# FHE-ACCELE/Homulator

Hardware: AMD Instinct MI355X
Metric: hmult+key-switch ops/sec (higher is better)
Workload: dtype u64

## Files before the change

homulator_amd/csrc/hm_backend.hip:

```cpp
#include <hip/hip_runtime.h>
#include <dlfcn.h>
#include <rccl/rccl.h>
#include <algorithm>
#include <cstdarg>
#include <cstdio>
#include <cstring>
#include <map>
#include <tuple>
#include <type_traits>
#include <utility>
#include <memory>
#include <stdexcept>
#include <string>
#include <vector>

#include "../../include/homulator_hip.h"
#include "hm_elem_core.h"
#include "hm_ip_core.h"
#include "hm_modarith.h"
#include "hm_ntt_core.h"
#include "hm_params.h"
#include "hm_caps.h"
#include "hm_launch.h"
#include "hm_bconv_plan.h"


__device__ __forceinline__ bool hm_block_map(uint32_t tiles_per_limb, uint32_t n_entries, uint32_t logG, uint32_t &entry, uint32_t &tile) {
  const uint32_t b = blockIdx.x, xcd = b & 7u, slot = b >> 3;
  const uint32_t per = tiles_per_limb << logG;
  const uint32_t grp = slot / per, within = slot % per;
  tile = within >> logG;
  entry = grp * (8u << logG) + (within & ((1u << logG) - 1u)) * 8u + xcd;
  return entry < n_entries;
}

#ifndef HM_ROW_WAVE_SYNC
#define HM_ROW_WAVE_SYNC 0
#endif
template <bool STRIDED>
__device__ __forceinline__ void hm_pass_sync(int nth) {
  if (STRIDED || !HM_ROW_WAVE_SYNC || nth == 0) __syncthreads();
  else { __builtin_amdgcn_fence(__ATOMIC_ACQ_REL, "wavefront"); __builtin_amdgcn_wave_barrier(); }
}

struct Geo16 {
  static constexpr int EPT = 16;
  typedef hm16::HmNttState State;
  template <int TL, int LOGR, bool STRIDED> static constexpr int ldsWords() { return hm16::HmLds<TL, LOGR, STRIDED>::WORDS; }
  template <int TL, int LOGR, bool STRIDED, bool INV, int MODE, int LDAUX, int STAUX, int EPICH, class... A>
  static __device__ __forceinline__ void phases(A &&...a) { hm16::hm_ntt_pass_phases<TL, LOGR, STRIDED, INV, MODE, LDAUX, STAUX, EPICH>(a...); }
};
struct Geo8 {
  static constexpr int EPT = 8;
  typedef hm8::HmNttState State;
  template <int TL, int LOGR, bool STRIDED> static constexpr int ldsWords() { return hm8::HmLds<TL, LOGR, STRIDED>::WORDS; }
  template <int TL, int LOGR, bool STRIDED, bool INV, int MODE, int LDAUX, int STAUX, int EPICH, class... A>
  static __device__ __forceinline__ void phases(A &&...a) { hm8::hm_ntt_pass_phases<TL, LOGR, STRIDED, INV, MODE, LDAUX, STAUX, EPICH>(a...); }
};
template <int LOGR, bool STRIDED, bool INV, int MODE, int LDAUX = 0, int STAUX = 0, int EPICH = HM_EPI_CHUNK, class GEO = Geo16, class PRE = HmNoPre>
__device__ __forceinline__ void hm_ntt_pass_run(const HmNttArgs &a, uint64_t *lds, uint32_t entry, uint32_t tile, int tid, PRE pre = PRE()) {
  constexpr int TL = HM_TL(STRIDED);
  const HmLimb lb = a.limb[entry];
  const uint32_t mod = lb.mod;
  const size_t N = (size_t)1 << a.logN;
  const uint64_t q = HM_CONST_MODS(a.mods)[mod].q;
  const HmW *twl = a.tw + (size_t)mod * N;
  const uint32_t s0 = STRIDED ? 0u : (a.logN - HM_ROW_LOG);
  const uint32_t prefix0 = STRIDED ? 0u : (tile << (TL - LOGR));
  const HmW *twt = STRIDED ? nullptr : a.twist + ((size_t)mod * (N >> HM_ROW_LOG) + prefix0) * 3;
  constexpr bool FIRST = (STRIDED != INV);
  const uint64_t *src = FIRST ? a.in + (size_t)lb.in * N : a.out + (size_t)lb.out * N;
  uint64_t *dst = a.out + (size_t)lb.out * N;

  HmTw sc = {0, 0};
  HmEpi ep = hm_epi_none();
  typedef const HmNttEntry __attribute__((address_space(4))) *ConstEntry;
  const ConstEntry entries = (ConstEntry)(uintptr_t)a.entry;
  if constexpr (MODE == 2) { sc.w = entries[entry].sc.w; sc.ws = entries[entry].sc.ws; ep.pack = entries[entry].pack; }
  if constexpr (MODE == 3 || MODE == 7) {
    const auto &en = entries[entry];
    sc.w = en.sc.w; sc.ws = en.sc.ws;
    ep.a = a.minuend + (size_t)lb.aux * N;
    ep.d = a.addend && en.alimb != HM_NTT_NONE ? a.addend + (size_t)en.alimb * N : nullptr;
    ep.dk.w = en.ak.w; ep.dk.ws = en.ak.ws;
    if constexpr (MODE == 7) { ep.g = en.galois; ep.logN = a.logN; }
  }
  if constexpr (MODE == 6) { ep.g = entries[entry].galois; ep.logN = a.logN; }
  if constexpr (MODE == 4) {
    const auto &en = entries[entry];
    ep.b = a.mix + (size_t)en.mixlimb * N;
    ep.bk.w = en.mixk.w; ep.bk.ws = en.mixk.ws;
  }
  typename GEO::State st;
  int nsync = 0;
  GEO::template phases<TL, LOGR, STRIDED, INV, MODE, LDAUX, STAUX, EPICH>(st, tid, lds, src, dst, tile, twl, twt, s0, prefix0, q, sc, ep,
                                                                           [&] { hm_pass_sync<STRIDED>(nsync++); }, pre);
}

template <int LOGR, bool STRIDED, bool INV, int MODE, class GEO = Geo16>
__device__ __forceinline__ void hm_ntt_pass_body(const HmNttArgs &a) {
  constexpr int TL = HM_TL(STRIDED);
  __shared__ __attribute__((aligned(16))) uint64_t lds[GEO::template ldsWords<TL, LOGR, STRIDED>()];
  uint32_t entry, tile;
  if (!hm_block_map(1u << (a.logN - TL), a.n_limbs, a.logG, entry, tile)) return;
  if (a.limb[entry].mod == HM_NTT_NONE) return;
#if defined(HM_ABL_EMPTY)
  return;
#endif
  hm_ntt_pass_run<LOGR, STRIDED, INV, MODE, 0, 0, HM_EPI_CHUNK, GEO>(a, lds, entry, tile, threadIdx.x);
}

#ifndef HM_NTT_MIN_WAVES
#define HM_NTT_MIN_WAVES 4
#endif
#ifndef HM_NTT_MIN_WAVES_COL
#define HM_NTT_MIN_WAVES_COL HM_NTT_MIN_WAVES
#endif
template <int LOGR, bool INV, int MODE>
__global__ void __launch_bounds__((1 << HM_TL_COL) / HM_EPT) __attribute__((amdgpu_waves_per_eu(HM_NTT_MIN_WAVES_COL))) k_ntt_col(HmNttArgs a) {
  hm_ntt_pass_body<LOGR, true, INV, MODE>(a);
}
template <bool INV, int MODE>
__global__ void __launch_bounds__((1 << HM_TL_ROW) / HM_EPT) __attribute__((amdgpu_waves_per_eu(HM_NTT_MIN_WAVES))) k_ntt_row(HmNttArgs a) {
  hm_ntt_pass_body<HM_ROW_LOG, false, INV, MODE>(a);
}

template <int LOG1, bool INV, int MODE>
__global__ void __launch_bounds__((1 << HM_TL_COL) / 8) k_ntt_col8(HmNttArgs a) {
  hm_ntt_pass_body<LOG1, true, INV, MODE, Geo8>(a);
}
template <bool INV, int MODE>
__global__ void __launch_bounds__((1 << HM_TL_ROW) / 8) k_ntt_row8(HmNttArgs a) {
  hm_ntt_pass_body<HM_ROW_LOG, false, INV, MODE, Geo8>(a);
}

struct HmLimbSync {
  unsigned long long w;
  unsigned long long pad[15];
};
struct HmNttSync {
  HmLimbSync fast[HM_NTT_MAX_ENTRIES];
  unsigned long long arrive2[HM_NTT_MAX_ENTRIES];
  unsigned done[HM_NTT_MAX_ENTRIES];
  unsigned xccmask[HM_NTT_MAX_ENTRIES];
  unsigned stats[4];
};
#define HM_SPIN_LIMIT (1u << 22)
#ifndef HM_OPAQUE_TID2
#define HM_OPAQUE_TID2 1
#endif
#ifndef HM_FUSED_IN_AUX
#define HM_FUSED_IN_AUX 0
#endif
#ifndef HM_FUSED_OUT_AUX
#define HM_FUSED_OUT_AUX 0
#endif
#ifndef HM_FUSED_MID_AUX
#define HM_FUSED_MID_AUX 16
#endif
__device__ __forceinline__ unsigned hm_xcc_id() {
  unsigned v;
  asm volatile("s_getreg_b32 %0, hwreg(HW_REG_XCC_ID, 0, 4)" : "=s"(v));
  return v & 7u;
}
__device__ __forceinline__ unsigned long long hm_l2_add(unsigned long long *p, unsigned long long v) {
  unsigned long long old;
  asm volatile("global_atomic_add_x2 %0, %1, %2, off sc0\n\ts_waitcnt vmcnt(0)" : "=v"(old) : "v"(p), "v"(v) : "memory");
  return old;
}
__device__ __forceinline__ void hm_l2_zero(unsigned long long *p) {
  unsigned long long old, z = 0;
  asm volatile("global_atomic_swap_x2 %0, %1, %2, off sc0\n\ts_waitcnt vmcnt(0)" : "=v"(old) : "v"(p), "v"(z) : "memory");
}
__device__ __forceinline__ void hm_l2_add_noret(unsigned long long *p, unsigned long long v) {
  asm volatile("global_atomic_add_x2 %0, %1, off" ::"v"(p), "v"(v) : "memory");
}
__device__ __forceinline__ void hm_limb_arrive(HmNttSync *ws, uint32_t entry, bool withhold) {
  asm volatile("s_waitcnt vmcnt(0)" ::: "memory");
  __syncthreads();
  if (threadIdx.x == 0 && !withhold) hm_l2_add_noret(&ws->fast[entry].w, 1ull);
}
__device__ __forceinline__ uint32_t hm_limb_wait(HmNttSync *ws, unsigned *err, uint32_t entry, uint32_t members, uint32_t *lds_flag, uint32_t spin_limit,
    uint32_t pretend_spread = 0, uint32_t tile = 0) {
  if (threadIdx.x == 0) {
    unsigned long long *w = &ws->fast[entry].w;
    uint32_t fast = 0;
    unsigned spins = 0;
// ... 769 lines not shown
  if (g->owner) {
    if (g->owner->live_graphs > 0) g->owner->live_graphs--;
    auto &v = g->owner->graphs;
    v.erase(std::remove(v.begin(), v.end(), g), v.end());
  }
  (void)hipGraphExecDestroy(g->exec);
  (void)hipGraphDestroy(g->graph);
  delete g;
}

extern "C" hm_status hm_timer_start(hm_ctx *c) {
  if (!c) return HM_ERR_ARG;
  HM_HIP(c, hipEventRecord(c->ev0, c->stream));
  return HM_OK;
}
extern "C" hm_status hm_timer_stop(hm_ctx *c, uint64_t *ns) {
  if (!c || !ns) return HM_ERR_ARG;
  HM_HIP(c, hipEventRecord(c->ev1, c->stream));
  HM_HIP(c, hipEventSynchronize(c->ev1));
  if (hm_status st = check_device_error(c)) return st;
  float ms = 0;
  HM_HIP(c, hipEventElapsedTime(&ms, c->ev0, c->ev1));
  *ns = (uint64_t)((double)ms * 1e6);
  return HM_OK;
}

static hm_status check_limbs(hm_ctx *c, const char *what, const uint32_t *l, uint32_t n) {
  for (uint32_t i = 0; l && i < n; ++i)
    if (l[i] > 0xFFFFu) return fail(c, HM_ERR_ARG, "%s: limb index %u exceeds 65535", what, l[i]);
  return HM_OK;
}
static hm_status check_mods(hm_ctx *c, const char *what, const uint32_t *m, uint32_t n) {
  if (!m) return fail(c, HM_ERR_ARG, "%s: mod_ids is null", what);
  for (uint32_t i = 0; i < n; ++i)
    if (m[i] >= c->P.L + c->P.K) return fail(c, HM_ERR_ARG, "%s: mod id %u out of range", what, m[i]);
  return HM_OK;
}

typedef void (*hm_ntt_kernel)(HmNttArgs);
typedef void (*hm_ntt_one_kernel)(HmNttArgs, HmNttFusedArgs);
struct HmNttKernels {
  hm_ntt_kernel first, second, first8, second8;
  hm_ntt_one_kernel one[2];
};
#define HM_NTT_FORMS 6
template <int LOG1>
static const HmNttKernels &ntt_kernels(int form) {
  static const HmNttKernels wide[HM_NTT_FORMS] = {
      {k_ntt_col<LOG1, false, 0>, k_ntt_row<false, 1>, nullptr, nullptr, {nullptr, nullptr}},
      {k_ntt_col<LOG1, false, 0>, k_ntt_row<false, 3>, nullptr, nullptr, {nullptr, nullptr}},
      {k_ntt_col<LOG1, false, 4>, k_ntt_row<false, 3>, nullptr, nullptr, {nullptr, nullptr}},
      {k_ntt_row<true, 0>, k_ntt_col<LOG1, true, 2>, nullptr, nullptr, {nullptr, nullptr}},
      {k_ntt_row<true, 6>, k_ntt_col<LOG1, true, 2>, nullptr, nullptr, {nullptr, nullptr}},
      {k_ntt_col<LOG1, false, 0>, k_ntt_row<false, 7>, nullptr, nullptr, {nullptr, nullptr}}};
  return wide[form];
}
template <int LOG1>
static const HmNttKernels &ntt_kernels_all(int form) {
  static const HmNttKernels both[HM_NTT_FORMS] = {
      {k_ntt_col<LOG1, false, 0>, k_ntt_row<false, 1>, k_ntt_col8<LOG1, false, 0>, k_ntt_row8<false, 1>, {k_ntt_fused8<LOG1, false, 0, 1, true>,
          k_ntt_fused8<LOG1, false, 0, 1, false>}},
      {k_ntt_col<LOG1, false, 0>, k_ntt_row<false, 3>, k_ntt_col8<LOG1, false, 0>, k_ntt_row8<false, 3>, {k_ntt_fused8<LOG1, false, 0, 3, true>,
          k_ntt_fused8<LOG1, false, 0, 3, false>}},
      {k_ntt_col<LOG1, false, 4>, k_ntt_row<false, 3>, k_ntt_col8<LOG1, false, 4>, k_ntt_row8<false, 3>, {k_ntt_fused8<LOG1, false, 4, 3, true>,
          k_ntt_fused8<LOG1, false, 4, 3, false>}},
      {k_ntt_row<true, 0>, k_ntt_col<LOG1, true, 2>, k_ntt_row8<true, 0>, k_ntt_col8<LOG1, true, 2>, {k_ntt_fused8<LOG1, true, 0, 2, true>,
          k_ntt_fused8<LOG1, true, 0, 2, false>}},
      {k_ntt_row<true, 6>, k_ntt_col<LOG1, true, 2>, k_ntt_row8<true, 6>, k_ntt_col8<LOG1, true, 2>, {k_ntt_fused8<LOG1, true, 6, 2, true>,
          k_ntt_fused8<LOG1, true, 6, 2, true>}},
      {k_ntt_col<LOG1, false, 0>, k_ntt_row<false, 7>, k_ntt_col8<LOG1, false, 0>, k_ntt_row8<false, 7>, {k_ntt_fused8<LOG1, false, 0, 7, true>,
          k_ntt_fused8<LOG1, false, 0, 7, false>}}};
  return both[form];
}
template <> const HmNttKernels &ntt_kernels<8>(int form) { return ntt_kernels_all<8>(form); }
template <> const HmNttKernels &ntt_kernels<7>(int form) { return ntt_kernels_all<7>(form); }

static uint32_t small_entries(const hm_ctx *c, uint32_t limbs16) {
  if (!hm_caps(c->P.logN).small_geometry) return 0;
  return std::min<uint32_t>(HM_NTT_MAX_ENTRIES, limbs16 << (16 - std::min(16u, c->P.logN)));
}
static uint32_t fused_small_entries(const hm_ctx *c) { return small_entries(c, c->fused_small); }

template <int LOG1>
static void launch_ntt(hm_ctx *c, const HmNttArgs &a, int form, bool firstPassOnly, bool secondPassOnly = false) {
  const HmNttKernels &K = ntt_kernels<LOG1>(form);
  const bool inverse = form == 3 || form == 4;
  const dim3 grid(a.n_limbs * (c->P.N >> HM_TL_ROW)), block16((1 << HM_TL_ROW) / HM_EPT), block8((1 << HM_TL_ROW) / 8);
  const bool small = K.first8 && c->small_ept8 && a.n_limbs <= small_entries(c, c->small_limbs);
  const bool col8 = small && (c->small_mode & 1), row8 = small && (c->small_mode & 2);
  const bool first8 = inverse ? row8 : col8, second8 = inverse ? col8 : row8;
  if (secondPassOnly) {
    hipLaunchKernelGGL(second8 ? K.second8 : K.second, grid, second8 ? block8 : block16, 0, c->stream, a);
    return;
  }
  if (firstPassOnly) {
    hipLaunchKernelGGL(K.first, grid, block16, 0, c->stream, a);
    return;
  }
  if (K.one[0] && a.n_limbs <= fused_small_entries(c) && a.logG == 0) {
    HmNttFusedArgs f = {c->ntt_ws, c->err_dev, c->fused_test_spread, c->fused_test_timeout ? 1u << 10 : HM_SPIN_LIMIT, c->fused_test_timeout};
#if defined(HM_FUSED_TRACE)
    f.trace = c->fused_trace;
#endif
    if (c->capturing) c->capture_has_fused = true;
    bool inPlace = a.in == a.out;
    for (uint32_t e = 0; inPlace && e < a.n_limbs; ++e) inPlace = a.limb[e].mod == HM_NTT_NONE || a.limb[e].in == a.limb[e].out;
    hipLaunchKernelGGL(K.one[inPlace ? 1 : 0], grid, block8, 0, c->stream, a, f);
    return;
  }
  hipLaunchKernelGGL(first8 ? K.first8 : K.first, grid, first8 ? block8 : block16, 0, c->stream, a);
  hipLaunchKernelGGL(second8 ? K.second8 : K.second, grid, second8 ? block8 : block16, 0, c->stream, a);
}

static hm_status device_table(hm_ctx *c, const void *data, size_t bytes, const void **out) {
  const std::string key(static_cast<const char *>(data), bytes);
  auto it = c->launch_tables.find(key);
  if (it == c->launch_tables.end()) {
    hipStreamCaptureStatus cs = hipStreamCaptureStatusNone;
    if (hipStreamIsCapturing(c->stream, &cs) == hipSuccess && cs != hipStreamCaptureStatusNone)
      return fail(c, HM_ERR_UNSUPPORTED, "a launch table is missing while the stream is capturing: run the plan once before hm_capture_begin");
    if (c->launch_tables.size() >= 1024 && c->live_graphs == 0 && !c->capturing) {
      HM_HIP(c, hipStreamSynchronize(c->stream));
      for (auto &kv : c->launch_tables) (void)hipFree(kv.second);
      c->launch_tables.clear();
    }
    void *dev = nullptr;
    HM_HIP(c, hipMalloc(&dev, bytes));
    HM_HIP(c, hipMemcpy(dev, data, bytes, hipMemcpyHostToDevice));
    it = c->launch_tables.emplace(key, dev).first;
  }
  *out = it->second;
  return HM_OK;
}
static hm_status ntt_table(hm_ctx *c, const std::vector<HmNttEntry> &tab, const HmNttEntry **out) {
  const void *p = nullptr;
  hm_status st = device_table(c, tab.data(), sizeof(HmNttEntry) * tab.size(), &p);
  *out = static_cast<const HmNttEntry *>(p);
  return st;
}

struct NttFused {
  const uint64_t *minuend = nullptr;
  const uint32_t *minuend_limbs = nullptr;
  const uint64_t *addend = nullptr;
  const uint32_t *addend_limbs = nullptr;
  const uint64_t *addend_k = nullptr;
  const uint64_t *mix = nullptr;
  const uint32_t *mix_limbs = nullptr;
  const uint64_t *mix_k = nullptr;
  const uint8_t *outPacked = nullptr;
  const uint32_t *inGalois = nullptr;
  const uint32_t *addGalois = nullptr;
  bool firstPassOnly = false;
  bool secondPassOnly = false;
};

static hm_status ntt_common(hm_ctx *c, const char *what, const uint64_t *in, const uint32_t *in_limbs, uint64_t *out,
                            const uint32_t *out_limbs, const uint32_t *mod_ids, uint32_t n, int inverse, const uint64_t *k,
                            const NttFused &f) {
  const bool fused = f.minuend != nullptr;
  hm_status st;
  if ((st = check_limbs(c, what, in_limbs, n)) || (st = check_limbs(c, what, out_limbs, n)) ||
      (st = check_limbs(c, what, f.minuend_limbs, n)) ||
      (st = check_limbs(c, what, f.mix_limbs, n)) || (st = check_mods(c, what, mod_ids, n)))
    return st;
  for (uint32_t g = 0; f.addend_limbs && g < n; ++g)
    if (f.addend_limbs[g] != HM_NO_LIMB && f.addend_limbs[g] >= 0xFFFFu) return fail(c, HM_ERR_ARG, "%s: addend limb index %u exceeds 65534", what,
        f.addend_limbs[g]);
  for (uint32_t g = 0; g < n; ++g) {
    const uint64_t q = c->P.mod[mod_ids[g]];
    if ((k && k[g] >= q) || (f.addend_k && f.addend_k[g] >= q) || (f.mix_k && f.mix_k[g] >= q))
      return fail(c, HM_ERR_ARG, "%s: constant [%u] is not reduced", what, g);
    if (f.addend_k && f.addend_k[g] == 0) return fail(c, HM_ERR_ARG, "%s: addend_k[%u] is zero (pass addend = NULL instead)", what, g);
  }
  bool anyInGalois = false, anyAddGalois = false;
  for (uint32_t g = 0; g < n; ++g) {
    const uint32_t gi = f.inGalois ? f.inGalois[g] : 0, ga = f.addGalois ? f.addGalois[g] : 0;
    if ((gi && (!(gi & 1) || gi >= 2 * c->P.N)) || (ga && (!(ga & 1) || ga >= 2 * c->P.N)))
      return fail(c, HM_ERR_ARG, "%s: Galois element [%u] is not an odd number below 2N", what, g);
    anyInGalois |= gi > 1; anyAddGalois |= ga > 1;
  }
  if (anyInGalois) {
    const int64_t g = hm_first_overlap(out, out_limbs, n, in, in_limbs, n, c->P.N, [&](uint32_t i) { return f.inGalois[i] > 1; });
    if (g >= 0) return fail(c, HM_ERR_ARG,
        "%s: limb-poly [%u] is read through an automorphism from a limb the call also writes (not in place, and not onto another entry's source)", what, (uint32_t)g);
  }
  if (anyInGalois && (!inverse || f.secondPassOnly)) return fail(c, HM_ERR_ARG, "%s: only the inverse transform reads its input through an automorphism", what);
  if (anyAddGalois && (!fused || f.mix || !f.addend)) return fail(c, HM_ERR_UNSUPPORTED,
      "%s: the addend is read through an automorphism by the fused forward transform without the mix prologue only", what);
  if (anyAddGalois) {
    const int64_t g = hm_first_overlap(out, out_limbs, n, f.addend, f.addend_limbs, n, c->P.N,
        [&](uint32_t i) { return f.addGalois[i] > 1 && !(f.addend_limbs && f.addend_limbs[i] == HM_NO_LIMB); });
    if (g >= 0) return fail(c, HM_ERR_ARG, "%s: the addend of limb-poly [%u] is read through an automorphism from a limb the call writes", what, (uint32_t)g);
  }
  HM_HIP(c, hipSetDevice(c->device));
  const bool oneLaunch = fused_small_entries(c) && !f.firstPassOnly && !f.secondPassOnly && (n + 7) / 8 * 8 <= fused_small_entries(c);
  std::vector<uint32_t> all(n);
  for (uint32_t i = 0; i < n; ++i) all[i] = i;
  const HmGrouping grouping = hm_group_by_modulus(mod_ids, all, hm_ntt_group_policy(oneLaunch));
  const auto &groups = grouping.groups;
  const uint32_t logG = grouping.logG, G = 1u << logG;
  const HmLaunchSplit parts = hm_launch_split((uint32_t)groups.size(), std::min<uint32_t>(HM_NTT_MAX_ENTRIES, c->ntt_launch_entries), G);
  for (uint32_t base = 0; base < groups.size(); base += parts.perLaunch) {
    const uint32_t ng = hm_launch_groups(parts, (uint32_t)groups.size(), base), cnt = hm_launch_entries(ng, G);
    std::vector<HmNttEntry> tab(cnt);
    memset(tab.data(), 0, sizeof(HmNttEntry) * cnt);
    HmNttArgs a;
    for (uint32_t e = 0; e < cnt; ++e) a.limb[e] = HmLimb{0, 0, (uint16_t)HM_NTT_NONE, 0};
    for (uint32_t kk = 0; kk < ng; ++kk) {
      for (uint32_t which = 0; which < G; ++which) {
        const int gi = groups[base + kk][which];
        if (gi < 0) continue;
        const uint32_t g = (uint32_t)gi, e = hm_entry_slot(kk, which, G), m = mod_ids[g];
        const uint64_t q = c->P.mod[m];
        HmNttEntry &t = tab[e];
        a.limb[e] = HmLimb{(uint16_t)limb_at(in_limbs, g), (uint16_t)limb_at(out_limbs, g), (uint16_t)m, 0};
        if (inverse) {
          uint64_t v = c->P.modc[m].ninv;
          if (k) v = hm::mulmod(v, k[g], q);
          t.sc = hm_kconst(v, q);
          t.pack = f.outPacked && f.outPacked[g] ? 1 : 0;
          if (anyInGalois) t.galois = f.inGalois[g] ? f.inGalois[g] : 1u;
        } else if (fused) {
          if (anyAddGalois) t.galois = f.addGalois[g] ? f.addGalois[g] : 1u;
          t.sc = hm_kconst(k[g], q);
          a.limb[e].aux = (uint16_t)limb_at(f.minuend_limbs, g);
          t.alimb = f.addend_limbs && f.addend_limbs[g] == HM_NO_LIMB ? (uint16_t)HM_NTT_NONE : (uint16_t)limb_at(f.addend_limbs, g);
          if (f.addend_k) t.ak = hm_kconst(f.addend_k[g], q);
          if (f.mix) {
            t.mixlimb = (uint16_t)limb_at(f.mix_limbs, g);
            t.mixk = hm_kconst(f.mix_k[g], q);
          }
        }
      }
    }
    const HmNttEntry *dtab = nullptr;
    if (inverse || fused) {
      if ((st = ntt_table(c, tab, &dtab))) return st;
    }
    a.in = in; a.out = out;
    a.tw = inverse ? c->d_tw_inv : c->d_tw_fwd;
    a.twist = inverse ? c->d_twist_inv : c->d_twist_fwd;
    a.mods = c->d_mods;
    a.entry = dtab;
    a.minuend = f.minuend; a.addend = f.addend; a.mix = f.mix;
    a.logN = c->P.logN; a.n_limbs = cnt; a.logG = logG;
    const int form = inverse ? (anyInGalois ? 4 : 3) : fused ? (f.mix ? 2 : anyAddGalois ? 5 : 1) : 0;
    static void (*const launch[])(hm_ctx *, const HmNttArgs &, int, bool, bool) = {launch_ntt<5>, launch_ntt<6>, launch_ntt<7>, launch_ntt<8>, launch_ntt<9>};
    const uint32_t log1 = c->P.logN - HM_ROW_LOG;
    if (log1 < 5 || log1 > 9) return fail(c, HM_ERR_UNSUPPORTED, "%s: logN %u", what, c->P.logN);
    launch[log1 - 5](c, a, form, f.firstPassOnly, f.secondPassOnly);
    HM_HIP(c, hipGetLastError());
  }
  return HM_OK;
}

extern "C" hm_status hm_ntt(hm_ctx *c, const uint64_t *in, const uint32_t *in_limbs, uint64_t *out,
                            const uint32_t *out_limbs, const uint32_t *mod_ids, uint32_t n, int inverse,
                            const uint64_t *scale) {
  if (!c) return HM_ERR_ARG;
  if (!in || !out) return fail(c, HM_ERR_ARG, "hm_ntt: null buffer");
  if (scale && !inverse) return fail(c, HM_ERR_ARG, "hm_ntt: scale is only defined for the inverse transform");
  return ntt_common(c, "hm_ntt", in, in_limbs, out, out_limbs, mod_ids, n, inverse, scale, NttFused{});
}

extern "C" hm_status hm_ntt_second_pass(hm_ctx *c, uint64_t *buf, const uint32_t *limbs, const uint32_t *mod_ids, uint32_t n, int inverse,
                                        const uint64_t *scale) {
  if (!c) return HM_ERR_ARG;
  if (!buf) return fail(c, HM_ERR_ARG, "hm_ntt_second_pass: null buffer");
  if (scale && !inverse) return fail(c, HM_ERR_ARG, "hm_ntt_second_pass: scale is only defined for the inverse transform");
  NttFused f;
  f.secondPassOnly = true;
  return ntt_common(c, "hm_ntt_second_pass", buf, limbs, buf, limbs, mod_ids, n, inverse, scale, f);
}

extern "C" hm_status hm_ntt_ex(hm_ctx *c, const hm_ntt_desc *d) {
  if (!c) return HM_ERR_ARG;
  if (!d || !d->out || (!d->in && !d->second_pass_only)) return fail(c, HM_ERR_ARG, "hm_ntt_ex: null buffer");
  if (d->scale && !d->inverse) return fail(c, HM_ERR_ARG, "hm_ntt_ex: scale is only defined for the inverse transform");
  if (d->out_packed && !d->inverse) return fail(c, HM_ERR_ARG, "hm_ntt_ex: out_packed is only defined for the inverse transform");
  NttFused f;
  f.secondPassOnly = d->second_pass_only != 0;
  f.outPacked = d->out_packed;
  f.inGalois = d->in_galois;
  if (d->in_galois && !d->inverse) return fail(c, HM_ERR_ARG, "hm_ntt_ex: in_galois is only defined for the inverse transform");
  if (f.secondPassOnly) return ntt_common(c, "hm_ntt_ex", d->out, d->out_limbs, d->out, d->out_limbs, d->mod_ids, d->n, d->inverse, d->scale, f);
  return ntt_common(c, "hm_ntt_ex", d->in, d->in_limbs, d->out, d->out_limbs, d->mod_ids, d->n, d->inverse, d->scale, f);
}

extern "C" hm_status hm_ntt_sub_scale(hm_ctx *c, const uint64_t *in, const uint32_t *in_limbs, const uint64_t *minuend,
                                      const uint32_t *minuend_limbs, const uint64_t *addend, const uint32_t *addend_limbs,
                                      uint64_t *out, const uint32_t *out_limbs, const uint32_t *mod_ids, uint32_t n,
                                      const uint64_t *k) {
  if (!c) return HM_ERR_ARG;
  if (!in || !out || !minuend || !k) return fail(c, HM_ERR_ARG, "hm_ntt_sub_scale: null argument");
  NttFused f;
  f.minuend = minuend; f.minuend_limbs = minuend_limbs; f.addend = addend; f.addend_limbs = addend_limbs;
  return ntt_common(c, "hm_ntt_sub_scale", in, in_limbs, out, out_limbs, mod_ids, n, 0, k, f);
}

struct BcolMix {
  const uint64_t *mix;
  const uint32_t *const *mix_limbs;
  const uint64_t *const *mix_k;
};
static hm_status bconv_col_launch(hm_ctx *c, const hm_bconv_desc *descs, uint32_t n_desc, const BcolMix *mix, uint32_t tile0 = 0, uint32_t n_tiles = 0);
extern "C" hm_status hm_ntt_mix_sub_scale(hm_ctx *c, const hm_ntt_fused_desc *d) {
  if (!c) return HM_ERR_ARG;
  if (!d || (!d->in && !d->n_conv) || !d->out || !d->minuend || !d->k) return fail(c, HM_ERR_ARG, "hm_ntt_mix_sub_scale: null argument");
  if ((d->mix != nullptr) != (d->mix_k != nullptr)) return fail(c, HM_ERR_ARG, "hm_ntt_mix_sub_scale: mix and mix_k go together");
  if (d->addend_k && !d->addend) return fail(c, HM_ERR_ARG, "hm_ntt_mix_sub_scale: addend_k without addend");
  NttFused f;
  f.minuend = d->minuend; f.minuend_limbs = d->minuend_limbs; f.addend = d->addend; f.addend_limbs = d->addend_limbs;
  f.addend_k = d->addend_k; f.mix = d->mix; f.mix_limbs = d->mix_limbs; f.mix_k = d->mix_k;
  f.addGalois = d->addend_galois;
  if (d->addend_galois && (d->n_conv || d->mix || !d->addend)) return fail(c, HM_ERR_UNSUPPORTED,
      "hm_ntt_mix_sub_scale: addend_galois needs an addend and combines with neither the mix prologue nor conversions inside the transform");
  if (!d->n_conv) return ntt_common(c, "hm_ntt_mix_sub_scale", d->in, d->in_limbs, d->out, d->out_limbs, d->mod_ids, d->n, 0, d->k, f);
  if (!d->conv) return fail(c, HM_ERR_ARG, "hm_ntt_mix_sub_scale: n_conv without descriptors");
  const uint32_t n = d->n;
  std::map<uint32_t, uint32_t> byOut;
  for (uint32_t i = 0; i < n; ++i)
    if (!byOut.emplace(limb_at(d->out_limbs, i), i).second) return fail(c, HM_ERR_ARG, "hm_ntt_mix_sub_scale: output limb %u appears twice",
        limb_at(d->out_limbs, i));
  std::vector<char> covered(n, 0);
  std::vector<std::vector<uint32_t>> mixLimbs(d->n_conv);
  std::vector<std::vector<uint64_t>> mixK(d->n_conv);
  std::vector<const uint32_t *> mlp(d->n_conv);
  std::vector<const uint64_t *> mkp(d->n_conv);
  for (uint32_t j = 0; j < d->n_conv; ++j) {
    const hm_bconv_desc &cv = d->conv[j];
    if (cv.out != d->out) return fail(c, HM_ERR_ARG, "hm_ntt_mix_sub_scale: conv[%u].out must be the output buffer", j);
    if (!cv.out_ids || cv.n_out == 0 || cv.n_out > HM_BCONV_MAX_OUT) return fail(c, HM_ERR_ARG, "hm_ntt_mix_sub_scale: conv[%u]: bad output basis", j);
    for (uint32_t t = 0; t < cv.n_out; ++t) {
// ... 422 lines not shown
```

homulator_amd/csrc/hm_launch.h:

```cpp
#pragma once
#include <algorithm>
#include <cstdint>
#include <map>
#include <vector>

static inline uint32_t limb_at(const uint32_t *l, uint32_t i) { return l ? l[i] : i; }

static inline uint32_t hm_entry_slot(uint32_t kk, uint32_t which, uint32_t G) { return (kk / 8) * 8 * G + which * 8 + (kk % 8); }

struct HmGroupPolicy {
  uint32_t defaultLogG, minLogG, maxLogG, sizeUnit;
};
#ifndef HM_NTT_MAX_LOGG
#define HM_NTT_MAX_LOGG 3
#endif
static inline HmGroupPolicy hm_ntt_group_policy(bool oneLaunch) { return HmGroupPolicy{oneLaunch ? 0u : 1u, 2, HM_NTT_MAX_LOGG, 64}; }
static inline HmGroupPolicy hm_nip_group_policy() { return HmGroupPolicy{0, 1, 3, 8}; }
struct HmGrouping {
  uint32_t logG = 0;
  std::vector<std::vector<int>> groups;
};
static inline HmGrouping hm_group_by_modulus(const uint32_t *mod_ids, const std::vector<uint32_t> &members, const HmGroupPolicy &p) {
  std::map<uint32_t, std::vector<int>> byMod;
  for (uint32_t i : members) byMod[mod_ids[i]].push_back((int)i);
  const size_t n = members.size();
  HmGrouping r;
  r.logG = p.defaultLogG;
  for (uint32_t lg = p.maxLogG; lg >= p.minLogG && lg > 0; --lg) {
    size_t full = 0;
    for (auto &kv : byMod) full += kv.second.size() >> lg << lg;
    if (full * 8 >= n * 7 && n >= ((size_t)p.sizeUnit << lg)) { r.logG = lg; break; }
  }
  const size_t G = (size_t)1 << r.logG;
  std::vector<int> rest;
  for (auto &kv : byMod) {
    auto &v = kv.second;
    size_t i = 0;
    for (; i + G <= v.size(); i += G) r.groups.emplace_back(v.begin() + i, v.begin() + i + G);
    rest.insert(rest.end(), v.begin() + i, v.end());
  }
  for (size_t i = 0; i < rest.size(); i += G) {
    std::vector<int> g(rest.begin() + i, rest.begin() + std::min(rest.size(), i + G));
    g.resize(G, -1);
    r.groups.push_back(g);
  }
  return r;
}
template <class Weight>
static inline void hm_sort_groups_heaviest_first(std::vector<std::vector<int>> &groups, Weight weight) {
  auto of = [&](const std::vector<int> &g) {
    uint32_t w = 0;
    for (int gi : g)
      if (gi >= 0) w += weight((uint32_t)gi);
    return w;
  };
  std::stable_sort(groups.begin(), groups.end(), [&](const std::vector<int> &a, const std::vector<int> &b) { return of(a) > of(b); });
}

struct HmLaunchSplit {
  uint32_t maxGroups, nLaunch, perLaunch;
};
static inline HmLaunchSplit hm_launch_split(uint32_t nGroups, uint32_t entryCap, uint32_t G) {
  HmLaunchSplit s;
  s.maxGroups = std::max(8u, entryCap / G / 8 * 8);
  s.nLaunch = (nGroups + s.maxGroups - 1) / s.maxGroups;
  s.perLaunch = s.nLaunch ? ((nGroups + s.nLaunch - 1) / s.nLaunch + 7) / 8 * 8 : 0;
  return s;
}
static inline uint32_t hm_launch_groups(const HmLaunchSplit &s, uint32_t nGroups, uint32_t base) { return std::min(s.perLaunch, nGroups - base); }
static inline uint32_t hm_launch_entries(uint32_t ng, uint32_t G) { return (ng + 7) / 8 * 8 * G; }

template <class Pick>
static inline int64_t hm_first_overlap(const void *ob, const uint32_t *ol, uint32_t no, const void *ib, const uint32_t *il, uint32_t ni, uint32_t N,
                                       Pick pick) {
  std::vector<int64_t> written(no);
  for (uint32_t i = 0; i < no; ++i) written[i] = limb_at(ol, i);
  std::sort(written.begin(), written.end());
  const int64_t lb = (int64_t)N * 8, base = (int64_t)(reinterpret_cast<intptr_t>(ib) - reinterpret_cast<intptr_t>(ob));
  for (uint32_t i = 0; i < ni; ++i) {
    if (!pick(i)) continue;
    const int64_t s = base + (int64_t)limb_at(il, i) * lb;
    const int64_t o0 = s >= 0 ? s / lb : -((-s + lb - 1) / lb);
    const int64_t o1 = o0 + (s != o0 * lb ? 1 : 0);
    auto it = std::lower_bound(written.begin(), written.end(), o0);
    if (it != written.end() && *it <= o1) return i;
  }
  return -1;
}
static inline bool hm_limbs_overlap(const void *ob, const uint32_t *ol, uint32_t no, const void *ib, const uint32_t *il, uint32_t ni, uint32_t N) {
  return hm_first_overlap(ob, ol, no, ib, il, ni, N, [](uint32_t) { return true; }) >= 0;
}
```

homulator_amd/csrc/hm_ntt_core.h:

```cpp
#pragma once
#include "hm_modarith.h"

#ifndef HM_TL_COL
#define HM_TL_COL 12
#endif
#ifndef HM_TL_ROW
#define HM_TL_ROW 12
#endif
#define HM_TL(STRIDED) ((STRIDED) ? HM_TL_COL : HM_TL_ROW)
#define HM_MAX_LIMBS 128
#ifndef HM_ROW_LOG
#define HM_ROW_LOG 8
#endif
#ifndef HM_TW_LDS_COL
#define HM_TW_LDS_COL 1
#endif
#ifndef HM_TW_LDS_ROW
#define HM_TW_LDS_ROW 1
#endif
#define HM_TW_IN_LDS(STRIDED) ((STRIDED) ? HM_TW_LDS_COL : HM_TW_LDS_ROW)
#ifndef HM_EPI_CHUNK
#define HM_EPI_CHUNK 2
#endif
#ifndef HM_EPI_FENCE
#define HM_EPI_FENCE 1
#endif
#ifndef HM_LATE_TW1
#define HM_LATE_TW1 1
#endif

struct HmLimb {
  uint16_t in, out, mod, aux;
};

struct HmNttEntry {
  uint16_t alimb, mixlimb;
  uint16_t pack;
  uint16_t pad;
  uint32_t galois;
  uint32_t pad1;
  HmTw sc;
  HmTw ak;
  HmTw mixk;
};
#define HM_NTT_NONE 0xFFFFu
#define HM_NTT_MAX_ENTRIES 448

struct HmNttArgs {
  const uint64_t *in;
  uint64_t *out;
  const HmW *tw;
  const HmW *twist;
  const HmMod *mods;
  const HmNttEntry *entry;
  const uint64_t *minuend, *addend, *mix;
  uint32_t logN;
  uint32_t n_limbs;
  uint32_t logG;
  HmLimb limb[HM_NTT_MAX_ENTRIES];
};
struct HmEpi {
  const uint64_t *a, *d;
  HmTw dk;
  const uint64_t *b;
  HmTw bk;
  uint32_t pack;
  uint32_t g, logN;
};
HM_HD HmEpi hm_epi_none() { return HmEpi{nullptr, nullptr, HmTw{0, 0}, nullptr, HmTw{0, 0}, 0, 0, 0}; }
HM_HD uint64_t hm_pack30(uint64_t x) { return (x & 0x3FFFFFFFull) | ((x >> 30) << 32); }
HM_HD uint64_t hm_unpack30(uint64_t p) { return (p & 0x3FFFFFFFull) | ((p >> 32) << 30); }

HM_HD uint32_t hm_brev(uint32_t x, uint32_t bits) {
#if defined(__HIP_DEVICE_COMPILE__)
  return __brev(x) >> (32 - bits);
#else
  uint32_t r = 0;
  for (uint32_t i = 0; i < bits; ++i) { r = (r << 1) | (x & 1); x >>= 1; }
  return r;
#endif
}
HM_HD uint32_t hm_auto_src(uint32_t i, uint32_t g, uint32_t logN) {
  uint32_t mask = (2u << logN) - 1;
  uint32_t e = (g * (2 * hm_brev(i, logN) + 1)) & mask;
  return hm_brev((e - 1) >> 1, logN);
}
HM_HD uint32_t hm_auto_inv(uint32_t g, uint32_t logN) {
  uint32_t v = g;
  for (int it = 0; it < 5; ++it) v *= 2u - g * v;
  return v & ((2u << logN) - 1);
}

HM_HD uint32_t hm_auto_pair(uint32_t i, uint32_t g, uint32_t logN, bool &swap) {
  const uint32_t s = hm_auto_src(i, g, logN);
  swap = s & 1u;
  return s & ~1u;
}

HM_HD void hm_ld2(const uint64_t *p, uint64_t &a, uint64_t &b) {
#if defined(__HIP_DEVICE_COMPILE__)
  const ulonglong2 t = *reinterpret_cast<const ulonglong2 *>(p);
  a = t.x; b = t.y;
#else
  a = p[0]; b = p[1];
#endif
}
HM_HD void hm_st2(uint64_t *p, uint64_t a, uint64_t b) {
#if defined(__HIP_DEVICE_COMPILE__)
  ulonglong2 t; t.x = a; t.y = b;
  *reinterpret_cast<ulonglong2 *>(p) = t;
#else
  p[0] = a; p[1] = b;
#endif
}

#if defined(__HIP_DEVICE_COMPILE__)
typedef unsigned hm_u32x4 __attribute__((ext_vector_type(4)));
HM_HD __amdgpu_buffer_rsrc_t hm_rsrc(const uint64_t *base) {
  return __builtin_amdgcn_make_buffer_rsrc(const_cast<uint64_t *>(base), 0, -1, 0x00020000);
}
#endif
HM_HD void hm_bld2(const uint64_t *base, uint32_t lane_bytes, uint64_t &v0, uint64_t &v1) {
#if defined(__HIP_DEVICE_COMPILE__)
  const hm_u32x4 t = __builtin_amdgcn_raw_buffer_load_b128(hm_rsrc(base), lane_bytes, 0, 0);
  v0 = (uint64_t)t.x | ((uint64_t)t.y << 32);
  v1 = (uint64_t)t.z | ((uint64_t)t.w << 32);
#else
  hm_ld2(base + (lane_bytes >> 3), v0, v1);
#endif
}
HM_HD void hm_bst2(uint64_t *base, uint32_t lane_bytes, uint64_t v0, uint64_t v1) {
#if defined(__HIP_DEVICE_COMPILE__)
  hm_u32x4 t;
  t.x = (unsigned)v0; t.y = (unsigned)(v0 >> 32); t.z = (unsigned)v1; t.w = (unsigned)(v1 >> 32);
  __builtin_amdgcn_raw_buffer_store_b128(t, hm_rsrc(base), lane_bytes, 0, 0);
#else
  hm_st2(base + (lane_bytes >> 3), v0, v1);
#endif
}
template <class G, int AUX = 0>
HM_HD void hm_gld2(const uint64_t *g, uint32_t tile, int tid, int a, uint64_t &v0, uint64_t &v1) {
// ... 72 lines not shown
```

Before: 5562.

## Group mix-epilogue NTT blocks by shared mix limb for cache reuse

For NTT passes with a MODE 4 mix epilogue, limbs are reordered so that blocks reading the same mix limb run as consecutive runs on the same XCD. This uses a new block map and grid size. The host side splits launches by mix-limb group and builds a separate entry table and argument struct for the first pass. The aim is to get L2/MALL reuse of the shared mix operand across limbs. The cost is padding entries and extra host-side table construction and uploads.

```diff
diff --git a/homulator_amd/csrc/hm_backend.hip b/homulator_amd/csrc/hm_backend.hip
--- a/homulator_amd/csrc/hm_backend.hip
+++ b/homulator_amd/csrc/hm_backend.hip
@@ -31,6 +31,14 @@
   const uint32_t grp = slot / per, within = slot % per;
   tile = within >> logG;
   entry = grp * (8u << logG) + (within & ((1u << logG) - 1u)) * 8u + xcd;
+  return entry < n_entries;
+}
+__device__ __forceinline__ bool hm_mix_block_map(uint32_t log_tiles, uint32_t n_entries, uint32_t run, uint32_t &entry, uint32_t &tile) {
+  const uint32_t b = blockIdx.x, xcd = b & 7u, slot = b >> 3;
+  const uint32_t rank = __builtin_amdgcn_readfirstlane(slot / run);
+  const uint32_t u = rank * 8u + xcd;
+  tile = u & ((1u << log_tiles) - 1u);
+  entry = (u >> log_tiles) * run + (slot - rank * run);
   return entry < n_entries;
 }
 
@@ -102,7 +110,9 @@
   constexpr int TL = HM_TL(STRIDED);
   __shared__ __attribute__((aligned(16))) uint64_t lds[GEO::template ldsWords<TL, LOGR, STRIDED>()];
   uint32_t entry, tile;
-  if (!hm_block_map(1u << (a.logN - TL), a.n_limbs, a.logG, entry, tile)) return;
+  if constexpr (MODE == 4) {
+    if (!hm_mix_block_map(a.logN - TL, a.n_limbs, a.mix_run, entry, tile)) return;
+  } else if (!hm_block_map(1u << (a.logN - TL), a.n_limbs, a.logG, entry, tile)) return;
   if (a.limb[entry].mod == HM_NTT_NONE) return;
 #if defined(HM_ABL_EMPTY)
   return;
@@ -1038,7 +1048,7 @@
 static uint32_t fused_small_entries(const hm_ctx *c) { return small_entries(c, c->fused_small); }
 
 template <int LOG1>
-static void launch_ntt(hm_ctx *c, const HmNttArgs &a, int form, bool firstPassOnly, bool secondPassOnly = false) {
+static void launch_ntt(hm_ctx *c, const HmNttArgs &a, const HmNttArgs *mixed, int form, bool firstPassOnly, bool secondPassOnly) {
   const HmNttKernels &K = ntt_kernels<LOG1>(form);
   const bool inverse = form == 3 || form == 4;
   const dim3 grid(a.n_limbs * (c->P.N >> HM_TL_ROW)), block16((1 << HM_TL_ROW) / HM_EPT), block8((1 << HM_TL_ROW) / 8);
@@ -1049,8 +1059,10 @@
     hipLaunchKernelGGL(second8 ? K.second8 : K.second, grid, second8 ? block8 : block16, 0, c->stream, a);
     return;
   }
+  const HmNttArgs &a1 = mixed ? *mixed : a;
+  const dim3 grid1(mixed ? hm_mix_grid(mixed->n_limbs / mixed->mix_run, c->P.N >> HM_TL_COL, mixed->mix_run) : grid.x);
   if (firstPassOnly) {
-    hipLaunchKernelGGL(K.first, grid, block16, 0, c->stream, a);
+    hipLaunchKernelGGL(K.first, grid1, block16, 0, c->stream, a1);
     return;
   }
   if (K.one[0] && a.n_limbs <= fused_small_entries(c) && a.logG == 0) {
@@ -1064,7 +1076,7 @@
     hipLaunchKernelGGL(K.one[inPlace ? 1 : 0], grid, block8, 0, c->stream, a, f);
     return;
   }
-  hipLaunchKernelGGL(first8 ? K.first8 : K.first, grid, first8 ? block8 : block16, 0, c->stream, a);
+  hipLaunchKernelGGL(first8 ? K.first8 : K.first, grid1, first8 ? block8 : block16, 0, c->stream, a1);
   hipLaunchKernelGGL(second8 ? K.second8 : K.second, grid, second8 ? block8 : block16, 0, c->stream, a);
 }
 
@@ -1151,23 +1163,21 @@
   }
   HM_HIP(c, hipSetDevice(c->device));
   const bool oneLaunch = fused_small_entries(c) && !f.firstPassOnly && !f.secondPassOnly && (n + 7) / 8 * 8 <= fused_small_entries(c);
-  std::vector<uint32_t> all(n);
-  for (uint32_t i = 0; i < n; ++i) all[i] = i;
-  const HmGrouping grouping = hm_group_by_modulus(mod_ids, all, hm_ntt_group_policy(oneLaunch));
-  const auto &groups = grouping.groups;
-  const uint32_t logG = grouping.logG, G = 1u << logG;
-  const HmLaunchSplit parts = hm_launch_split((uint32_t)groups.size(), std::min<uint32_t>(HM_NTT_MAX_ENTRIES, c->ntt_launch_entries), G);
-  for (uint32_t base = 0; base < groups.size(); base += parts.perLaunch) {
-    const uint32_t ng = hm_launch_groups(parts, (uint32_t)groups.size(), base), cnt = hm_launch_entries(ng, G);
+  const std::vector<HmNttLaunch> launches = hm_ntt_launches(mod_ids, f.mix_limbs, f.mix != nullptr, n, hm_ntt_group_policy(oneLaunch),
+      std::min<uint32_t>(HM_NTT_MAX_ENTRIES, c->ntt_launch_entries));
+  for (const HmNttLaunch &l : launches) {
+    const uint32_t logG = l.logG, G = 1u << logG, ng = (uint32_t)l.groups.size(), cnt = hm_launch_entries(ng, G);
     std::vector<HmNttEntry> tab(cnt);
     memset(tab.data(), 0, sizeof(HmNttEntry) * cnt);
     HmNttArgs a;
     for (uint32_t e = 0; e < cnt; ++e) a.limb[e] = HmLimb{0, 0, (uint16_t)HM_NTT_NONE, 0};
+    std::vector<uint32_t> slotOf(n, 0);
     for (uint32_t kk = 0; kk < ng; ++kk) {
       for (uint32_t which = 0; which < G; ++which) {
-        const int gi = groups[base + kk][which];
+        const int gi = l.groups[kk][which];
         if (gi < 0) continue;
         const uint32_t g = (uint32_t)gi, e = hm_entry_slot(kk, which, G), m = mod_ids[g];
+        slotOf[g] = e;
         const uint64_t q = c->P.mod[m];
         HmNttEntry &t = tab[e];
         a.limb[e] = HmLimb{(uint16_t)limb_at(in_limbs, g), (uint16_t)limb_at(out_limbs, g), (uint16_t)m, 0};
@@ -1200,12 +1210,28 @@
     a.mods = c->d_mods;
     a.entry = dtab;
     a.minuend = f.minuend; a.addend = f.addend; a.mix = f.mix;
-    a.logN = c->P.logN; a.n_limbs = cnt; a.logG = logG;
+    a.logN = c->P.logN; a.n_limbs = cnt; a.logG = logG; a.mix_run = 0;
+    HmNttArgs am;
+    if (f.mix) {
+      const uint32_t cm = (uint32_t)l.mix.rec.size();
+      std::vector<HmNttEntry> tabm(cm);
+      memset(tabm.data(), 0, sizeof(HmNttEntry) * cm);
+      memcpy(&am, &a, offsetof(HmNttArgs, limb));
+      for (uint32_t e = 0; e < cm; ++e) {
+        const int gi = l.mix.rec[e];
+        am.limb[e] = gi < 0 ? HmLimb{0, 0, (uint16_t)HM_NTT_NONE, 0} : a.limb[slotOf[gi]];
+        if (gi >= 0) tabm[e] = tab[slotOf[gi]];
+      }
+      const HmNttEntry *dtabm = nullptr;
+      if ((st = ntt_table(c, tabm, &dtabm))) return st;
+      am.entry = dtabm; am.n_limbs = cm; am.mix_run = l.mix.run;
+    }
     const int form = inverse ? (anyInGalois ? 4 : 3) : fused ? (f.mix ? 2 : anyAddGalois ? 5 : 1) : 0;
-    static void (*const launch[])(hm_ctx *, const HmNttArgs &, int, bool, bool) = {launch_ntt<5>, launch_ntt<6>, launch_ntt<7>, launch_ntt<8>, launch_ntt<9>};
+    static void (*const launch[])(hm_ctx *, const HmNttArgs &, const HmNttArgs *, int, bool, bool) = {launch_ntt<5>, launch_ntt<6>, launch_ntt<7>, launch_ntt<8>,
+        launch_ntt<9>};
     const uint32_t log1 = c->P.logN - HM_ROW_LOG;
     if (log1 < 5 || log1 > 9) return fail(c, HM_ERR_UNSUPPORTED, "%s: logN %u", what, c->P.logN);
-    launch[log1 - 5](c, a, form, f.firstPassOnly, f.secondPassOnly);
+    launch[log1 - 5](c, a, f.mix ? &am : nullptr, form, f.firstPassOnly, f.secondPassOnly);
     HM_HIP(c, hipGetLastError());
   }
   return HM_OK;
diff --git a/homulator_amd/csrc/hm_launch.h b/homulator_amd/csrc/hm_launch.h
--- a/homulator_amd/csrc/hm_launch.h
+++ b/homulator_amd/csrc/hm_launch.h
@@ -7,6 +7,9 @@
 static inline uint32_t limb_at(const uint32_t *l, uint32_t i) { return l ? l[i] : i; }
 
 static inline uint32_t hm_entry_slot(uint32_t kk, uint32_t which, uint32_t G) { return (kk / 8) * 8 * G + which * 8 + (kk % 8); }
+static inline uint32_t hm_entry_block(uint32_t e, uint32_t tile, uint32_t tiles, uint32_t G) {
+  return (((e / (8 * G)) * tiles + tile) * G + (e / 8) % G) * 8 + e % 8;
+}
 
 struct HmGroupPolicy {
   uint32_t defaultLogG, minLogG, maxLogG, sizeUnit;
@@ -70,6 +73,91 @@
 static inline uint32_t hm_launch_groups(const HmLaunchSplit &s, uint32_t nGroups, uint32_t base) { return std::min(s.perLaunch, nGroups - base); }
 static inline uint32_t hm_launch_entries(uint32_t ng, uint32_t G) { return (ng + 7) / 8 * 8 * G; }
 
+#define HM_MIX_RUN_MAX 128
+static inline uint32_t hm_mix_block(uint32_t grp, uint32_t member, uint32_t tile, uint32_t tiles, uint32_t run) {
+  const uint32_t u = grp * tiles + tile;
+  return ((u / 8) * run + member) * 8 + (u % 8);
+}
+static inline uint32_t hm_mix_grid(uint32_t nGroups, uint32_t tiles, uint32_t run) { return (nGroups * tiles + 7) / 8 * 8 * run; }
+struct HmMixOrder {
+  uint32_t run = 0;
+  std::vector<int> rec;
+};
+static inline HmMixOrder hm_mix_order(const uint32_t *mix_limbs, const std::vector<uint32_t> &members, uint32_t entryCap) {
+  std::map<uint32_t, std::vector<int>> byMix;
+  for (uint32_t i : members) byMix[limb_at(mix_limbs, i)].push_back((int)i);
+  std::vector<std::vector<int>> groups;
+  for (auto &kv : byMix)
+    for (size_t i = 0; i < kv.second.size(); i += HM_MIX_RUN_MAX)
+      groups.emplace_back(kv.second.begin() + i, kv.second.begin() + std::min(kv.second.size(), i + HM_MIX_RUN_MAX));
+  HmMixOrder o;
+  for (auto &g : groups) o.run = std::max<uint32_t>(o.run, (uint32_t)g.size());
+  if (groups.size() * o.run > entryCap) {
+    o.run = 1;
+    for (uint32_t i : members) o.rec.push_back((int)i);
+    return o;
+  }
+  for (auto &g : groups) {
+    o.rec.insert(o.rec.end(), g.begin(), g.end());
+    o.rec.resize(o.rec.size() + (o.run - g.size()), -1);
+  }
+  return o;
+}
+
+struct HmNttLaunch {
+  uint32_t logG = 0;
+  std::vector<std::vector<int>> groups;
+  HmMixOrder mix;
+};
+static inline std::vector<HmNttLaunch> hm_ntt_launches(const uint32_t *mod_ids, const uint32_t *mix_limbs, bool mixed, uint32_t n, const HmGroupPolicy &p,
+                                                       uint32_t entryCap) {
+  auto split = [&](const std::vector<uint32_t> &members) {
+    std::vector<HmNttLaunch> r;
+    const HmGrouping g = hm_group_by_modulus(mod_ids, members, p);
+    const uint32_t G = 1u << g.logG, nGroups = (uint32_t)g.groups.size();
+    const HmLaunchSplit parts = hm_launch_split(nGroups, entryCap, G);
+    for (uint32_t base = 0; base < nGroups; base += parts.perLaunch) {
+      HmNttLaunch l;
+      l.logG = g.logG;
+      l.groups.assign(g.groups.begin() + base, g.groups.begin() + base + hm_launch_groups(parts, nGroups, base));
+      if (mixed) {
+        std::vector<uint32_t> live;
+        for (auto &grp : l.groups)
+          for (int gi : grp)
+            if (gi >= 0) live.push_back((uint32_t)gi);
+        std::sort(live.begin(), live.end());
+        l.mix = hm_mix_order(mix_limbs, live, entryCap);
+      }
+      r.push_back(std::move(l));
+    }
+    return r;
+  };
+  std::vector<uint32_t> all(n);
+  for (uint32_t i = 0; i < n; ++i) all[i] = i;
+  if (!mixed || n == 0) return split(all);
+  std::map<uint32_t, std::vector<uint32_t>> byMix;
+  for (uint32_t i = 0; i < n; ++i) byMix[limb_at(mix_limbs, i)].push_back(i);
+  std::vector<HmNttLaunch> r;
+  for (size_t k = (n + entryCap - 1) / entryCap;; ++k) {
+    r.clear();
+    bool whole = true;
+    std::vector<uint32_t> part;
+    size_t seen = 0, done = 0;
+    for (auto it = byMix.begin(); it != byMix.end(); ++it) {
+      part.insert(part.end(), it->second.begin(), it->second.end());
+      seen += it->second.size();
+      if (seen * k >= (done + 1) * (size_t)n || std::next(it) == byMix.end()) {
+        std::vector<HmNttLaunch> v = split(part);
+        whole = whole && v.size() == 1;
+        for (auto &l : v) r.push_back(std::move(l));
+        part.clear();
+        ++done;
+      }
+    }
+    if (whole || k >= byMix.size()) return r;
+  }
+}
+
 template <class Pick>
 static inline int64_t hm_first_overlap(const void *ob, const uint32_t *ol, uint32_t no, const void *ib, const uint32_t *il, uint32_t ni, uint32_t N,
                                        Pick pick) {
diff --git a/homulator_amd/csrc/hm_ntt_core.h b/homulator_amd/csrc/hm_ntt_core.h
--- a/homulator_amd/csrc/hm_ntt_core.h
+++ b/homulator_amd/csrc/hm_ntt_core.h
@@ -57,6 +57,7 @@
   uint32_t logN;
   uint32_t n_limbs;
   uint32_t logG;
+  uint32_t mix_run;
   HmLimb limb[HM_NTT_MAX_ENTRIES];
 };
 struct HmEpi {
```

Result: slower. 5475 (-1.6%).
